# facebookresearch/Active-3D-Vision-and-Touch

Measured on AMD Instinct MI355X. Metric: mesh-recon iters/sec (fwd+bwd, 2562-vert GCN + 10k-pt Chamfer) at bs=64, higher is better.
Workload: dtype f32; 1 GPU; icosphere-4 template (2562 verts, 5120 faces), 3-stage GCN 20x300 cut 0.33, bs=64/GPU, 10000-pt Chamfer x3 draws, Adam, ellipsoid clouds (BASELINE.json configs[1]); global_batch=64, parallelism=dp1

## Files before the change

### active-3d-vision-and-touch_amd/csrc/gcn_csrq.hip

```cpp
#include "common.h"
#include "kernels.h"

namespace a3vt {

using f32x4 = __attribute__((ext_vector_type(4))) float;

constexpr int kCsrqThreads = 512;
constexpr int kHeavyDegQ = 64;
constexpr int kEllW = 8;

using i32x2 = __attribute__((ext_vector_type(2))) int;
__device__ __forceinline__ float bits_to_f32(int x) { return __builtin_bit_cast(float, x); }
__device__ __forceinline__ int f32_to_bits(float x) { return __builtin_bit_cast(int, x); }
__global__ void csr_ell_build_kernel(const int32_t *__restrict__ rowptr, const int32_t *__restrict__ colidx,
                                     const float *__restrict__ val, int n_vert, i32x2 *__restrict__ ell,
                                     int32_t *__restrict__ degs) {
  const int v = blockIdx.x * blockDim.x + threadIdx.x;
  if (v >= n_vert) return;
  const int e0 = rowptr[v], n = rowptr[v + 1] - e0;
  degs[v] = n;
#pragma unroll
  for (int j = 0; j < kEllW; ++j)
    ell[(size_t)j * n_vert + v] = j < n ? i32x2{colidx[e0 + j], f32_to_bits(val[e0 + j])} : i32x2{n_vert, 0};
}
size_t csrq_ell_ints(int n_vert) { return (size_t)n_vert * (2 * kEllW + 1) + 64; }
int launch_csrq_ell(const int32_t *rowptr, const int32_t *col, const float *val, int n_vert, int32_t *ell, hipStream_t s) {
  A3VT_LAUNCH(csr_ell_build_kernel, dim3(cdiv(n_vert, 256)), dim3(256), 0, s, rowptr, col, val, n_vert,
              reinterpret_cast<i32x2 *>(ell), ell + (size_t)n_vert * 2 * kEllW);
  A3VT_CHECK_LAUNCH();
  return 0;
}

#ifdef A3VT_DBG_CSRQ_STAMPS
__device__ unsigned long long g_csrq_stamps[2 * 2 * 256 * 8 * 4];
#define CSRQ_STAMP(qi, k)                                                                                     \
  do {                                                                                                        \
    if (threadIdx.x == 0 && blockIdx.x < 256 && (qi) < 8) {                                                   \
      const int i_ = ((MODE * 256 + blockIdx.x) * 8 + (qi)) * 4 + (k);                                        \
      g_csrq_stamps[i_] = __builtin_amdgcn_s_memrealtime();                                                   \
      g_csrq_stamps[2 * 256 * 8 * 4 + i_] = __builtin_amdgcn_s_memtime();                                     \
    }                                                                                                         \
  } while (0)
#else
#define CSRQ_STAMP(qi, k) do { } while (0)
#endif

template <int MODE, int VPT>
__global__ __launch_bounds__(kCsrqThreads) void csrq_kernel(const float *__restrict__ srcq, int nq, int parts,
                                                            const float *__restrict__ bias, int c,
                                                            const int32_t *__restrict__ rowptr,
                                                            const int32_t *__restrict__ colidx,
                                                            const float *__restrict__ val, int n_vert, int batch,
                                                            float *__restrict__ dst, int nq_dst,
                                                            uint8_t *__restrict__ signq, int relu, int heavy_thresh,
                                                            float *__restrict__ db_slab,
                                                            const int32_t *__restrict__ ellbuf) {
  extern __shared__ __attribute__((aligned(16))) float lds_raw[];
  __shared__ float red[2][kCsrqThreads / 64][4];
  const i32x2 *ell = reinterpret_cast<const i32x2 *>(ellbuf);
  const int32_t *degs = ellbuf + (size_t)n_vert * 2 * kEllW;
  f32x4 *tile0 = reinterpret_cast<f32x4 *>(lds_raw);
  const int xcd = blockIdx.x & 7, loc = blockIdx.x >> 3;
  const int jm = loc / parts, part = loc - jm * parts;
  const int b = xcd + 8 * jm;
  if (b >= batch) return;
  const int q_lo = part * nq / parts, q_hi = (part + 1) * nq / parts;
  if (q_lo >= q_hi) return;
  CSRQ_STAMP(7, 0);

  int vv[VPT], dg[VPT];
  bool on[VPT];
  int cj[VPT][kEllW];
  float wj[VPT][kEllW];
#pragma unroll
  for (int k = 0; k < VPT; ++k) {
    const int v = threadIdx.x + k * kCsrqThreads;
    on[k] = v < n_vert;
    vv[k] = on[k] ? v : n_vert - 1;
#ifdef A3VT_DBG_CSRQ_NOINDEX
    dg[k] = 6;
#pragma unroll
    for (int j = 0; j < kEllW; ++j) cj[k][j] = (vv[k] + j * 37) % n_vert, wj[k][j] = 0.125f;
#else
    dg[k] = degs[vv[k]];
#pragma unroll
    for (int j = 0; j < kEllW; ++j) {
      const i32x2 e = ell[(size_t)j * n_vert + vv[k]];
      const int e0 = e[0], e1 = e[1];
      cj[k][j] = e0;
      wj[k][j] = bits_to_f32(e1);
    }
#endif
  }

  auto fetch = [&](int q, int k, f32x4 &v4, unsigned &bits) {
    const size_t plane = ((size_t)b * nq + q) * n_vert;
    v4 = reinterpret_cast<const f32x4 *>(srcq)[plane + vv[k]];
    bits = MODE == 1 ? signq[plane + vv[k]] : 0u;
  };
  auto park = [&](f32x4 *tile, int q, int k, f32x4 v4, unsigned bits) {
    if (MODE == 1) {
#pragma unroll
      for (int t = 0; t < 4; ++t) v4[t] = ((bits >> t) & 1u) ? v4[t] : 0.f;
    }
    (void)q;
    tile[vv[k]] = v4;
  };

  if (threadIdx.x < 2) tile0[(size_t)threadIdx.x * (n_vert + 1) + n_vert] = f32x4{0.f, 0.f, 0.f, 0.f};
  {
    f32x4 v4[VPT];
    unsigned bits[VPT];
#pragma unroll
    for (int k = 0; k < VPT; ++k) fetch(q_lo, k, v4[k], bits[k]);
#pragma unroll
    for (int k = 0; k < VPT; ++k) park(tile0, q_lo, k, v4[k], bits[k]);
  }
  __syncthreads();

  for (int q = q_lo; q < q_hi; ++q) {
    CSRQ_STAMP(q - q_lo, 0);
    const int par = (q - q_lo) & 1;
    const f32x4 *tile = tile0 + (size_t)par * (n_vert + 1);
    f32x4 *tnext = tile0 + (size_t)(par ^ 1) * (n_vert + 1);
    const int ch = q * 4;
    const size_t plane = ((size_t)b * nq + q) * n_vert;
    const int qn = q + 1 < q_hi ? q + 1 : q;
    f32x4 nv4[VPT];
    unsigned nbits[VPT];
#pragma unroll
    for (int k = 0; k < VPT; ++k) fetch(qn, k, nv4[k], nbits[k]);
    f32x4 bs = {0.f, 0.f, 0.f, 0.f};
    if (MODE == 0) {
#pragma unroll
      for (int t = 0; t < 4; ++t)
        if (ch + t < c) bs[t] = bias[ch + t];
    }
    f32x4 bsum = {0.f, 0.f, 0.f, 0.f};
#pragma unroll
    for (int k = 0; k < VPT; ++k) {
      __builtin_amdgcn_sched_barrier(0);
      const int v = vv[k];
      const f32x4 own = tile[v];
      if (MODE == 1) {
#pragma unroll
        for (int t = 0; t < 4; ++t) bsum[t] += on[k] ? own[t] : 0.f;
      }
      f32x4 acc = {0.f, 0.f, 0.f, 0.f};
#pragma unroll
      for (int j = 0; j < kEllW; ++j) {
#ifdef A3VT_DBG_CSRQ_NOGATHER
        acc[j & 3] += wj[k][j] * (float)cj[k][j];
#else
        {
          const f32x4 r = tile[cj[k][j]];
          const float w = wj[k][j];
          acc[0] = __builtin_fmaf(w, r[0], acc[0]);
          acc[1] = __builtin_fmaf(w, r[1], acc[1]);
          acc[2] = __builtin_fmaf(w, r[2], acc[2]);
          acc[3] = __builtin_fmaf(w, r[3], acc[3]);
        }
#endif
      }
      if (dg[k] > kEllW && dg[k] <= heavy_thresh) {
        const int ea = rowptr[v];
        for (int e = ea + kEllW; e < ea + dg[k]; ++e) {
          const f32x4 r = tile[colidx[e]];
          const float w = val[e];
#pragma unroll
          for (int t = 0; t < 4; ++t) acc[t] = __builtin_fmaf(w, r[t], acc[t]);
        }
      }
      if (!on[k] || dg[k] > heavy_thresh) continue;
      f32x4 o;
      if (MODE == 0) {
        unsigned bits = 0;
#pragma unroll
        for (int t = 0; t < 4; ++t) {
          const float pre = ch + t < c ? acc[t] + bs[t] : own[t];
          o[t] = (pre > 0.f || !relu) ? pre : 0.f;
          bits |= (pre > 0.f ? 1u : 0u) << t;
        }
        if (signq) signq[plane + v] = (uint8_t)bits;
      } else {
#pragma unroll
        for (int t = 0; t < 4; ++t) o[t] = ch + t < c ? acc[t] : own[t];
      }
      *reinterpret_cast<f32x4 *>(dst + ((((size_t)b * nq_dst + q) * n_vert) + v) * 4) = o;
    }
    __builtin_amdgcn_sched_barrier(0);
    CSRQ_STAMP(q - q_lo, 1);
    if (MODE == 1) {
#pragma unroll
      for (int t = 0; t < 4; ++t) bsum[t] = wave_sum(bsum[t]);
      if ((threadIdx.x & 63) == 0) {
#pragma unroll
        for (int t = 0; t < 4; ++t) red[par][threadIdx.x >> 6][t] = bsum[t];
      }
    }
    if (q + 1 < q_hi) {
#pragma unroll
      for (int k = 0; k < VPT; ++k) park(tnext, q + 1, k, nv4[k], nbits[k]);
    }
    CSRQ_STAMP(q - q_lo, 2);
    __syncthreads();
    if (MODE == 1 && threadIdx.x < 4) {
      float sacc = 0.f;
#pragma unroll
      for (int w = 0; w < kCsrqThreads / 64; ++w) sacc += red[par][w][threadIdx.x];
      db_slab[(size_t)b * (nq * 4) + ch + threadIdx.x] = sacc;
    }
    CSRQ_STAMP(q - q_lo, 3);
  }
}

template <int MODE>
__global__ __launch_bounds__(256) void csrq_heavy_kernel(const float *__restrict__ srcq, int nq,
                                                         const float *__restrict__ bias, int c,
                                                         const int32_t *__restrict__ rowptr,
                                                         const int32_t *__restrict__ colidx,
                                                         const float *__restrict__ val, int n_vert, int batch,
                                                         const int32_t *__restrict__ heavy, float *__restrict__ dst,
                                                         int nq_dst, uint8_t *__restrict__ signq, int relu) {
  __shared__ f32x4 red[8][32];
  const int hl = threadIdx.x & 31, sub = threadIdx.x >> 5;
  const int count = heavy[0];
  const bool on = hl < nq;
  const int ch = hl * 4;
  for (long long item = blockIdx.x; item < (long long)count * batch; item += gridDim.x) {
    const int v = heavy[64 + (int)(item % count)];
    const long long b = item / count;
    const size_t plane = ((size_t)b * nq + (on ? hl : 0)) * n_vert;
    const f32x4 *src = reinterpret_cast<const f32x4 *>(srcq) + plane;
    const int e0 = rowptr[v], e1 = rowptr[v + 1];
    const int per = ((e1 - e0 + 7) / 8 + 3) & ~3;
    const int s0 = min(e1, e0 + sub * per), s1 = min(e1, s0 + per);
    f32x4 acc = {0.f, 0.f, 0.f, 0.f};
    if (on) {
      for (int e = s0; e < s1; ++e) {
        const int cc = colidx[e];
        f32x4 r = src[cc];
        if (MODE == 1) {
          const unsigned bits = signq[plane + cc];
#pragma unroll
          for (int t = 0; t < 4; ++t) r[t] = ((bits >> t) & 1u) ? r[t] : 0.f;
        }
#pragma unroll
        for (int t = 0; t < 4; ++t) acc[t] = __builtin_fmaf(val[e], r[t], acc[t]);
      }
    }
    red[sub][hl] = acc;
    __syncthreads();
    if (sub == 0 && on) {
      f32x4 a = red[0][hl];
#pragma unroll
      for (int r = 1; r < 8; ++r) a += red[r][hl];
      f32x4 own = src[v];
      f32x4 o;
      if (MODE == 0) {
        unsigned bits = 0;
#pragma unroll
        for (int t = 0; t < 4; ++t) {
          const float pre = ch + t < c ? a[t] + bias[ch + t] : own[t];
          o[t] = (pre > 0.f || !relu) ? pre : 0.f;
          bits |= (pre > 0.f ? 1u : 0u) << t;
        }
        if (signq) signq[plane + v] = (uint8_t)bits;
      } else {
        const unsigned bits = signq[plane + v];
#pragma unroll
        for (int t = 0; t < 4; ++t) {
          own[t] = ((bits >> t) & 1u) ? own[t] : 0.f;
          o[t] = ch + t < c ? a[t] : own[t];
        }
      }
      *reinterpret_cast<f32x4 *>(dst + ((((size_t)b * nq_dst + hl) * n_vert) + v) * 4) = o;
    }
    __syncthreads();
  }
}

int csrq_max_degree() { return kEllW; }
#ifdef A3VT_DBG_CSRQ_STAMPS
}
extern "C" int a3vt_dbg_csrq_stamps(unsigned long long *host_dst) {
  return (int)hipMemcpyFromSymbol(host_dst, HIP_SYMBOL(a3vt::g_csrq_stamps), sizeof(unsigned long long) * 2 * 2 * 256 * 8 * 4);
}
namespace a3vt {
#endif
bool csrq_fits(int n_vert, int cut_len) {
  return cut_len > 0 && pad4(cut_len) <= 128 && n_vert <= 6 * kCsrqThreads && ((size_t)n_vert + 1) * 32 <= 158 * 1024;
}

template <int MODE, int VPT>
static int launch_csrq_vpt(const float *srcq, int nq, const float *bias, int c, const int32_t *rowptr, const int32_t *col,
                           const float *val, const int32_t *heavy, const int32_t *ell, int n_vert, int batch, float *dst,
                           int nq_dst, uint8_t *signq, int relu, float *db_slab, hipStream_t s) {
  const size_t shmem = ((size_t)n_vert + 1) * 32;
  static OncePerDevice once;
  once.run([] {
    (void)hipFuncSetAttribute((const void *)csrq_kernel<MODE, VPT>, hipFuncAttributeMaxDynamicSharedMemorySize, 158 * 1024);
  });
  int parts = 256 / (((batch + 7) / 8) * 8);
  parts = parts < 1 ? 1 : parts > nq ? nq : parts;
  const int grid = 8 * ((batch + 7) / 8) * parts;
  A3VT_LAUNCH((csrq_kernel<MODE, VPT>), dim3(grid), dim3(kCsrqThreads), shmem, s, srcq, nq, parts, bias, c, rowptr, col, val,
              n_vert, batch, dst, nq_dst, signq, relu, heavy ? kHeavyDegQ : 0x7fffffff, db_slab, ell);
  A3VT_CHECK_LAUNCH();
  return 0;
}

template <int MODE>
static int launch_csrq(const float *srcq, const float *bias, int c, const int32_t *rowptr, const int32_t *col,
                       const float *val, const int32_t *heavy, const int32_t *ell, int n_vert, int batch, float *dst,
                       int nq_dst, uint8_t *signq, int relu, float *db_slab, hipStream_t s) {
  const int nq = pad4(c) / 4;
  if (!csrq_fits(n_vert, c) || nq_dst < nq || (MODE == 1 && (!signq || !db_slab))) {
    set_error("csrq: n_vert=%d c=%d output planes=%d unsupported", n_vert, c, nq_dst);
    return -1;
  }
  int rc;
  if (n_vert <= 4 * kCsrqThreads)
    rc = launch_csrq_vpt<MODE, 4>(srcq, nq, bias, c, rowptr, col, val, heavy, ell, n_vert, batch, dst, nq_dst, signq, relu, db_slab, s);
  else
    rc = launch_csrq_vpt<MODE, 6>(srcq, nq, bias, c, rowptr, col, val, heavy, ell, n_vert, batch, dst, nq_dst, signq, relu, db_slab, s);
  if (rc) return rc;
  if (heavy) {
    A3VT_LAUNCH(csrq_heavy_kernel<MODE>, dim3(2048), dim3(256), 0, s, srcq, nq, bias, c, rowptr, col, val, n_vert, batch,
                heavy, dst, nq_dst, signq, relu);
    A3VT_CHECK_LAUNCH();
  }
  return 0;
}

int launch_csrq_fwd(const float *zq, const float *bias, int c, const int32_t *rowptr, const int32_t *col,
                    const float *val, const int32_t *heavy, const int32_t *ell, int n_vert, int batch, float *yq,
                    int yq_quads, uint8_t *signq, int relu, hipStream_t s) {
  return launch_csrq<0>(zq, bias, c, rowptr, col, val, heavy, ell, n_vert, batch, yq, yq_quads, signq, relu, nullptr, s);
}
int launch_csrq_bwd(const float *gq, int c, const int32_t *rowptrT, const int32_t *colT, const float *valT,
                    const int32_t *heavyT, const int32_t *ellT, int n_vert, int batch, float *dzaq,
                    const uint8_t *signq, float *db_slab, hipStream_t s) {
  return launch_csrq<1>(gq, nullptr, c, rowptrT, colT, valT, heavyT, ellT, n_vert, batch, dzaq, pad4(c) / 4,
                        const_cast<uint8_t *>(signq), 0, db_slab, s);
}

}
```

Measured before the change: 22.02 iters/s.

## Compact ELL index with two-weight encoding and split remainder quads across blocks

The ELL build now also emits a compact per-vertex record: eight 16-bit column indices packed in an int4, plus an int4 holding two distinct weight values and a bitmask selecting between them. Regular vertices load these two int4s instead of eight int2 entries, and a wave falls back to the full ELL only when some lane is irregular. This cuts index-load traffic and register setup at kernel start. Quad partitioning also changes: each block gets an equal number of full quads, and leftover quads are shared by several blocks that split the vertex slices by wave, so no block carries an extra quad. The cost is redundant tile loads for shared quads, more indexing logic, and a narrower code path that relies on the mesh having few distinct weights per row and fewer than 65536 vertices.

```diff
diff --git a/active-3d-vision-and-touch_amd/csrc/gcn_csrq.hip b/active-3d-vision-and-touch_amd/csrc/gcn_csrq.hip
--- a/active-3d-vision-and-touch_amd/csrc/gcn_csrq.hip
+++ b/active-3d-vision-and-touch_amd/csrc/gcn_csrq.hip
@@ -10,23 +10,47 @@
 constexpr int kEllW = 8;
 
 using i32x2 = __attribute__((ext_vector_type(2))) int;
+using i32x4 = __attribute__((ext_vector_type(4))) int;
 __device__ __forceinline__ float bits_to_f32(int x) { return __builtin_bit_cast(float, x); }
 __device__ __forceinline__ int f32_to_bits(float x) { return __builtin_bit_cast(int, x); }
+constexpr int kCsrqIrregular = -1;
 __global__ void csr_ell_build_kernel(const int32_t *__restrict__ rowptr, const int32_t *__restrict__ colidx,
                                      const float *__restrict__ val, int n_vert, i32x2 *__restrict__ ell,
-                                     int32_t *__restrict__ degs) {
+                                     int32_t *__restrict__ degs, i32x4 *__restrict__ ccol, i32x4 *__restrict__ cw) {
   const int v = blockIdx.x * blockDim.x + threadIdx.x;
   if (v >= n_vert) return;
   const int e0 = rowptr[v], n = rowptr[v + 1] - e0;
   degs[v] = n;
-#pragma unroll
-  for (int j = 0; j < kEllW; ++j)
-    ell[(size_t)j * n_vert + v] = j < n ? i32x2{colidx[e0 + j], f32_to_bits(val[e0 + j])} : i32x2{n_vert, 0};
-}
-size_t csrq_ell_ints(int n_vert) { return (size_t)n_vert * (2 * kEllW + 1) + 64; }
+  const int wa = n > 0 ? f32_to_bits(val[e0]) : 0;
+  int wb = wa, mask = 0;
+  bool regular = n <= kEllW && n_vert <= 0xffff;
+  int packed[kEllW / 2] = {};
+#pragma unroll
+  for (int j = 0; j < kEllW; ++j) {
+    const int cj = j < n ? colidx[e0 + j] : n_vert;
+    const int wj = j < n ? f32_to_bits(val[e0 + j]) : 0;
+    if (j < n && wj != wa) {
+      if (wb == wa) wb = wj;
+      regular = regular && wj == wb;
+      mask |= 1 << j;
+    }
+    ell[(size_t)j * n_vert + v] = i32x2{cj, wj};
+    packed[j / 2] |= (cj & 0xffff) << (16 * (j & 1));
+  }
+  regular = regular && wa >= 0 && wa < 0x7f800000 && wb >= 0 && wb < 0x7f800000;
+#ifdef A3VT_DBG_CSRQ_NOCOMPACT
+  regular = false;
+#endif
+  ccol[v] = i32x4{packed[0], packed[1], packed[2], packed[3]};
+  cw[v] = regular ? i32x4{wa, wb, mask, 0} : i32x4{kCsrqIrregular, 0, 0, 0};
+}
+__host__ __device__ static size_t csrq_compact_off(int n_vert) { return ((size_t)n_vert * (2 * kEllW + 1) + 3) & ~(size_t)3; }
+size_t csrq_ell_ints(int n_vert) { return csrq_compact_off(n_vert) + (size_t)n_vert * 8 + 64; }
 int launch_csrq_ell(const int32_t *rowptr, const int32_t *col, const float *val, int n_vert, int32_t *ell, hipStream_t s) {
+  int32_t *cmp = ell + csrq_compact_off(n_vert);
   A3VT_LAUNCH(csr_ell_build_kernel, dim3(cdiv(n_vert, 256)), dim3(256), 0, s, rowptr, col, val, n_vert,
-              reinterpret_cast<i32x2 *>(ell), ell + (size_t)n_vert * 2 * kEllW);
+              reinterpret_cast<i32x2 *>(ell), ell + (size_t)n_vert * 2 * kEllW, reinterpret_cast<i32x4 *>(cmp),
+              reinterpret_cast<i32x4 *>(cmp + (size_t)n_vert * 4));
   A3VT_CHECK_LAUNCH();
   return 0;
 }
@@ -59,13 +83,20 @@
   __shared__ float red[2][kCsrqThreads / 64][4];
   const i32x2 *ell = reinterpret_cast<const i32x2 *>(ellbuf);
   const int32_t *degs = ellbuf + (size_t)n_vert * 2 * kEllW;
+  const i32x4 *ccol = reinterpret_cast<const i32x4 *>(ellbuf + csrq_compact_off(n_vert));
+  const i32x4 *cw = reinterpret_cast<const i32x4 *>(ellbuf + csrq_compact_off(n_vert) + (size_t)n_vert * 4);
   f32x4 *tile0 = reinterpret_cast<f32x4 *>(lds_raw);
   const int xcd = blockIdx.x & 7, loc = blockIdx.x >> 3;
   const int jm = loc / parts, part = loc - jm * parts;
   const int b = xcd + 8 * jm;
   if (b >= batch) return;
-  const int q_lo = part * nq / parts, q_hi = (part + 1) * nq / parts;
-  if (q_lo >= q_hi) return;
+  const int full = nq / parts, rem = nq - full * parts;
+  const int nmine = full + (rem > 0 ? 1 : 0);
+  const int qs = rem > 0 ? full * parts + part % rem : 0;
+  const int sh = rem > 0 ? part / rem : 0;
+  const int nsh = rem > 0 ? (parts - 1 - part % rem) / rem + 1 : 1;
+  const int wave = __builtin_amdgcn_readfirstlane(threadIdx.x >> 6);
+  auto quad_of = [&](int i) { return i < full ? part * full + i : qs; };
   CSRQ_STAMP(7, 0);
 
   int vv[VPT], dg[VPT];
@@ -77,33 +108,17 @@
     const int v = threadIdx.x + k * kCsrqThreads;
     on[k] = v < n_vert;
     vv[k] = on[k] ? v : n_vert - 1;
-#ifdef A3VT_DBG_CSRQ_NOINDEX
-    dg[k] = 6;
-#pragma unroll
-    for (int j = 0; j < kEllW; ++j) cj[k][j] = (vv[k] + j * 37) % n_vert, wj[k][j] = 0.125f;
-#else
-    dg[k] = degs[vv[k]];
-#pragma unroll
-    for (int j = 0; j < kEllW; ++j) {
-      const i32x2 e = ell[(size_t)j * n_vert + vv[k]];
-      const int e0 = e[0], e1 = e[1];
-      cj[k][j] = e0;
-      wj[k][j] = bits_to_f32(e1);
-    }
-#endif
-  }
-
+  }
   auto fetch = [&](int q, int k, f32x4 &v4, unsigned &bits) {
     const size_t plane = ((size_t)b * nq + q) * n_vert;
     v4 = reinterpret_cast<const f32x4 *>(srcq)[plane + vv[k]];
     bits = MODE == 1 ? signq[plane + vv[k]] : 0u;
   };
-  auto park = [&](f32x4 *tile, int q, int k, f32x4 v4, unsigned bits) {
+  auto park = [&](f32x4 *tile, int k, f32x4 v4, unsigned bits) {
     if (MODE == 1) {
 #pragma unroll
       for (int t = 0; t < 4; ++t) v4[t] = ((bits >> t) & 1u) ? v4[t] : 0.f;
     }
-    (void)q;
     tile[vv[k]] = v4;
   };
 
@@ -112,20 +127,63 @@
     f32x4 v4[VPT];
     unsigned bits[VPT];
 #pragma unroll
-    for (int k = 0; k < VPT; ++k) fetch(q_lo, k, v4[k], bits[k]);
-#pragma unroll
-    for (int k = 0; k < VPT; ++k) park(tile0, q_lo, k, v4[k], bits[k]);
+    for (int k = 0; k < VPT; ++k) fetch(quad_of(0), k, v4[k], bits[k]);
+
+#ifdef A3VT_DBG_CSRQ_NOINDEX
+#pragma unroll
+    for (int k = 0; k < VPT; ++k) {
+      dg[k] = 6;
+#pragma unroll
+      for (int j = 0; j < kEllW; ++j) cj[k][j] = (vv[k] + j * 37) % n_vert, wj[k][j] = 0.125f;
+    }
+#else
+    i32x4 pc[VPT], pw[VPT];
+#pragma unroll
+    for (int k = 0; k < VPT; ++k) pc[k] = ccol[vv[k]], pw[k] = cw[vv[k]];
+    bool irr = false;
+#pragma unroll
+    for (int k = 0; k < VPT; ++k) {
+      const int wa = pw[k][0], wb = pw[k][1], mask = pw[k][2];
+#pragma unroll
+      for (int j = 0; j < kEllW; ++j) {
+        const int pj = pc[k][j / 2];
+        cj[k][j] = (j & 1) ? (int)((unsigned)pj >> 16) : (pj & 0xffff);
+        wj[k][j] = bits_to_f32(((mask >> j) & 1) ? wb : wa);
+      }
+      dg[k] = 0;
+      irr = irr || wa == kCsrqIrregular;
+    }
+    if (__builtin_amdgcn_ballot_w64(irr) != 0) {
+#pragma unroll
+      for (int k = 0; k < VPT; ++k) {
+        const bool ik = pw[k][0] == kCsrqIrregular;
+        const int d = degs[vv[k]];
+        dg[k] = ik ? d : 0;
+#pragma unroll
+        for (int j = 0; j < kEllW; ++j) {
+          const i32x2 e = ell[(size_t)j * n_vert + vv[k]];
+          const int e0 = e[0], e1 = e[1];
+          cj[k][j] = ik ? e0 : cj[k][j];
+          wj[k][j] = ik ? bits_to_f32(e1) : wj[k][j];
+        }
+      }
+    }
+#endif
+#pragma unroll
+    for (int k = 0; k < VPT; ++k) park(tile0, k, v4[k], bits[k]);
   }
   __syncthreads();
 
-  for (int q = q_lo; q < q_hi; ++q) {
-    CSRQ_STAMP(q - q_lo, 0);
-    const int par = (q - q_lo) & 1;
+  for (int i = 0; i < nmine; ++i) {
+    CSRQ_STAMP(i, 0);
+    const int q = quad_of(i);
+    const bool shared = i >= full;
+    const int par = i & 1;
     const f32x4 *tile = tile0 + (size_t)par * (n_vert + 1);
     f32x4 *tnext = tile0 + (size_t)(par ^ 1) * (n_vert + 1);
     const int ch = q * 4;
     const size_t plane = ((size_t)b * nq + q) * n_vert;
-    const int qn = q + 1 < q_hi ? q + 1 : q;
+    const int qn = i + 1 < nmine ? quad_of(i + 1) : q;
     f32x4 nv4[VPT];
     unsigned nbits[VPT];
 #pragma unroll
@@ -146,6 +204,7 @@
 #pragma unroll
         for (int t = 0; t < 4; ++t) bsum[t] += on[k] ? own[t] : 0.f;
       }
+      if (shared && (wave + k) % nsh != sh) continue;
       f32x4 acc = {0.f, 0.f, 0.f, 0.f};
 #pragma unroll
       for (int j = 0; j < kEllW; ++j) {
@@ -189,7 +248,7 @@
       *reinterpret_cast<f32x4 *>(dst + ((((size_t)b * nq_dst + q) * n_vert) + v) * 4) = o;
     }
     __builtin_amdgcn_sched_barrier(0);
-    CSRQ_STAMP(q - q_lo, 1);
+    CSRQ_STAMP(i, 1);
     if (MODE == 1) {
 #pragma unroll
       for (int t = 0; t < 4; ++t) bsum[t] = wave_sum(bsum[t]);
@@ -198,19 +257,19 @@
         for (int t = 0; t < 4; ++t) red[par][threadIdx.x >> 6][t] = bsum[t];
       }
     }
-    if (q + 1 < q_hi) {
-#pragma unroll
-      for (int k = 0; k < VPT; ++k) park(tnext, q + 1, k, nv4[k], nbits[k]);
-    }
-    CSRQ_STAMP(q - q_lo, 2);
+    if (i + 1 < nmine) {
+#pragma unroll
+      for (int k = 0; k < VPT; ++k) park(tnext, k, nv4[k], nbits[k]);
+    }
+    CSRQ_STAMP(i, 2);
     __syncthreads();
-    if (MODE == 1 && threadIdx.x < 4) {
+    if (MODE == 1 && threadIdx.x < 4 && (!shared || sh == 0)) {
       float sacc = 0.f;
 #pragma unroll
       for (int w = 0; w < kCsrqThreads / 64; ++w) sacc += red[par][w][threadIdx.x];
       db_slab[(size_t)b * (nq * 4) + ch + threadIdx.x] = sacc;
     }
-    CSRQ_STAMP(q - q_lo, 3);
+    CSRQ_STAMP(i, 3);
   }
 }
 
```

Measured after the change: 22.14 iters/s (median of 6 runs). No clear change (+0.5%).
